# UltronAI/Depth-VO-Feat

Measured on AMD Instinct MI355X. Metric: KITTI 256x832 stereo-seq samples/sec fwd+bwd, higher is better.
Workload: dtype f32

## Files before the change

depth-vo-feat_amd/csrc/conv.hip:

```cpp
#include "dvf_common.h"
#include "conv_op.h"
#include "conv_pipe_host.h"
#include "conv_gather.h"
#include "conv_wgrad.h"
#include "wgrad_pipe.h"

namespace {

__device__ __forceinline__ float act_grad(float g, float yv, int act, float alpha, float beta) {
    if (act == DVF_ACT_RELU) return (yv > 0.f) ? g : 0.f;
    if (act == DVF_ACT_SIGMOID_AFFINE) {
        const float sg = (yv - beta) / alpha;
        return g * alpha * sg * (1.f - sg);
    }
    return g;
}

template <bool VEC>
__global__ __launch_bounds__(256) void act_bwd_kernel(const float *__restrict__ dy, const float *__restrict__ y,
                                                      float *__restrict__ dpre, float *dbias, int C, int HW, int act,
                                                      float alpha, float beta, int chunks, float *part = nullptr, int nper = 0) {
    __shared__ float red[4];
    const int plane = blockIdx.x / chunks, chunk = blockIdx.x - plane * chunks;
    const int c = plane % C;
// ... 224 lines not shown
    else rc = launch_gather_ck<1, 1>(a, pl, st);
    if (rc) return rc;
    dvf_plan_note(DVF_K_GATHER, pl.MT, pl.NT, 1, 2 * pl.CKH, 0, a.KS, 1, 1, 256, (int)pl.lds, a.out_mode | (a.ncls << 4));
    return finish_output(a, pl.reduce_kpar, ws, io.out, st);
}

enum FwdDirect { FWD_NONE, FWD_HEAD, FWD_HEAD_WIDE, FWD_DCONVT };
FwdDirect fwd_direct(const dvf_conv_desc *d, int nseg) {
    if (dvf_head_applicable(d, nseg)) return FWD_HEAD;
    if (dvf_head_wide_applicable(d, nseg)) return FWD_HEAD_WIDE;
    if (dvf_dconvt_applicable(d, nseg)) return FWD_DCONVT;
    return FWD_NONE;
}

int fwd_unpacked(const dvf_conv_desc *d, const ConvOp &op, const ConvIO &io, const int *seg_channels, int nseg, const float *w,
                 float *ws, int64_t ws_floats, hipStream_t st) {
    switch (fwd_direct(d, nseg)) {
        case FWD_HEAD: return dvf_head_fwd(d, io.in[0], w, io.bias, io.out, st);
        case FWD_HEAD_WIDE: return dvf_head_fwd_segs(d, io.in, seg_channels, nseg, w, io.bias, io.out, st);
        case FWD_DCONVT: return dvf_dconvt_fwd(d, io.in[0], w, io.bias, io.out, st);
        case FWD_NONE: break;
    }
    GatherPlan pl;
    const int rc = plan_gather(op, pl);
    return rc ? rc : run_gather(op, pl, io, w, ws, ws_floats, st);
}

int dgrad_unpacked(const dvf_conv_desc *d, const ConvOp &op, const ConvIO &io, const float *w, float *ws, int64_t ws_floats,
                   hipStream_t st) {
    if (dvf_head_seg_dgrad_applicable(d, op.M))
        return dvf_head_seg_dgrad(d, io.in[0], w, io.out, op.m_base, op.M, st, io.mask);
    GatherPlan pl;
    const int rc = plan_gather(op, pl);
    return rc ? rc : run_gather(op, pl, io, w, ws, ws_floats, st);
}

int64_t unpacked_ws_floats(const ConvOp &op, bool direct) {
    if (direct) return 0;
    GatherPlan pl;
    const int rc = plan_gather(op, pl);
    return rc ? rc : pl.ws_floats;
}

struct DgradSeg {
    int s, off;
    ConvOp op;
    bool packed;
    PipePlan plan;
    int64_t packed_off;
};

template <class F>
int for_each_dgrad_seg(const dvf_conv_desc *d, const int *seg_channels, int nseg, bool use_pipe, F visit) {
    DgradSeg v;
    v.off = 0; v.packed_off = 0;
    for (v.s = 0; v.s < nseg; ++v.s) {
        int rc = make_dgrad_op(d, v.off, seg_channels[v.s], v.op);
        v.packed = false;
        if (use_pipe) {
            if (rc) return rc;
            rc = plan_pipe(v.op, v.plan);
            if (rc && rc != DVF_ERR_UNSUPPORTED) return rc;
            v.packed = !rc;
        }
        rc = visit(v);
        if (rc) return rc;
        if (v.packed) v.packed_off += v.plan.packed_floats;
        v.off += seg_channels[v.s];
    }
    return DVF_OK;
}

int64_t conv_sizes(const dvf_conv_desc *d, const int *seg_channels, int nseg, int op_kind, bool want_ws) {
    int rc = check_desc(d);
    if (rc) return rc;
    rc = check_segs(d, seg_channels, nseg);
    if (rc) return rc;
    if (op_kind == 0) {
        if (!want_ws && dvf_dconvt_applicable(d, nseg)) return DVF_ERR_UNSUPPORTED;
        ConvOp op;
        PipePlan pl;
        rc = make_fwd_op(d, seg_channels, nseg, op);
        if (rc) return rc;
        rc = plan_pipe(op, pl);
        if (rc == DVF_ERR_UNSUPPORTED && want_ws) return unpacked_ws_floats(op, fwd_direct(d, nseg) != FWD_NONE);
        return rc ? rc : (want_ws ? pl.ws_floats : pl.packed_floats);
    }
    if (op_kind != 1) return DVF_ERR_INVALID_ARG;
    int64_t total = 0, wmax = 0;
    int nsup = 0;
    rc = for_each_dgrad_seg(d, seg_channels, nseg, true, [&](const DgradSeg &v) -> int {
        int64_t wf = 0;
        if (v.packed) {
            total += v.plan.packed_floats;
            wf = v.plan.ws_floats;
            ++nsup;
        } else if (want_ws) {
            wf = unpacked_ws_floats(v.op, dvf_head_seg_dgrad_applicable(d, v.op.M));
            if (wf < 0) return (int)wf;
        }
        wmax = wf > wmax ? wf : wmax;
        return DVF_OK;
    });
    if (rc) return rc;
    if (!nsup && !want_ws) return DVF_ERR_UNSUPPORTED;
    return want_ws ? wmax : total;
}

WgradArgs wgrad_args(const dvf_conv_desc *d, const float *const *in_segs, const int *seg_channels, int s, const float *dpre,
                     float *dw) {
    int off = 0;
    for (int i = 0; i < s; ++i) off += seg_channels[i];
    const int segc = s < 0 ? d->C_in : seg_channels[s];
    WgradArgs a{};
    a.KK = d->KH * d->KW; a.KH = d->KH; a.KW = d->KW; a.N = d->N; a.S = d->stride; a.pad = d->pad; a.G = dw;
    if (!d->transposed) {
        a.P = dpre; a.PCtot = d->C_out; a.m_base = 0; a.M = d->C_out; a.GH = d->H_out; a.GW = d->W_out;
        a.Q = s < 0 ? nullptr : in_segs[s]; a.QCtot = segc; a.q_base = 0; a.Cq = segc; a.QH = d->H_in; a.QW = d->W_in;
        a.g_mstride = (int64_t)d->C_in * a.KK; a.g_mbase = 0; a.g_cbase = off;
    } else {
        a.P = in_segs[s]; a.PCtot = segc; a.m_base = 0; a.M = segc; a.GH = d->H_in; a.GW = d->W_in;
        a.Q = dpre; a.QCtot = d->C_out; a.q_base = 0; a.Cq = d->C_out; a.QH = d->H_out; a.QW = d->W_out;
        a.g_mstride = (int64_t)d->C_out * a.KK; a.g_mbase = off; a.g_cbase = 0;
    }
    return a;
}

struct WgradPipePlan {
    WgpArgs w;
    int MT, NTW, TILE, nblocks;
    size_t lds;
    int64_t ws_floats;
};

int plan_wgrad_pipe(const WgradArgs &o, const int *qsegc, int nseg, bool aligned16, bool want_bias, WgradPipePlan &pl) {
    static const bool off = dvf_tune("DVF_WG_PIPE") && atoi(dvf_tune("DVF_WG_PIPE")) == 0;
    if (off) return DVF_ERR_UNSUPPORTED;
    const int T = o.KH * o.KW;
    if ((o.S != 1 && o.S != 2) || T > 128 || o.pad < 0 || o.pad > 4) return DVF_ERR_UNSUPPORTED;
    if ((int64_t)o.N * o.PCtot * o.GH * o.GW * 4 >= ((int64_t)1 << 31) - 16 ||
        nseg < 1 || nseg > DVF_MAX_SEGS)
        return DVF_ERR_UNSUPPORTED;
    WgpArgs &w = pl.w;
    w = WgpArgs{};
    for (int s = 0; s < nseg; ++s) {
        if ((int64_t)o.N * qsegc[s] * o.QH * o.QW * 4 >= ((int64_t)1 << 31) - 16) return DVF_ERR_UNSUPPORTED;
        w.segC[s] = qsegc[s];
    }
    w.nseg = nseg;
    w.PCtot = o.PCtot; w.m_base = o.m_base; w.M = o.M; w.Cq = o.Cq;
    w.g_mstride = o.g_mstride; w.g_mbase = o.g_mbase; w.g_cbase = o.g_cbase; w.KK = o.KK; w.KH = o.KH; w.KW = o.KW;
    w.N = o.N; w.GH = o.GH; w.GW = o.GW; w.QH = o.QH; w.QW = o.QW; w.S = o.S; w.pad = o.pad;
    w.XA = (o.pad + 3) & ~3;
    w.RSq = roundup(w.XA + (WGP_BW - 1) * o.S + o.KW - o.pad, 4);
    w.PHq = (WGP_BH - 1) * o.S + o.KH;
    w.x4 = (o.GW % 4 == 0 && o.QW % 4 == 0 && aligned16) ? 1 : 0;
    if (const char *e = dvf_tune("DVF_WG_X4")) w.x4 = w.x4 && atoi(e) != 0;
    const int piece = w.x4 ? 256 : 64;
    w.NPIq = cdiv(w.PHq * w.RSq, piece);
    if (w.NPIq > WGP_MAXQ) return DVF_ERR_UNSUPPORTED;
    w.PSq = w.NPIq * piece + 4;
    static const bool no16 = dvf_tune("DVF_WG_TILE16") && atoi(dvf_tune("DVF_WG_TILE16")) == 0;
    double best_cost = 1e30;
    int TILE = 0, MT = 0, NTW = 0, CK = 0;
    for (int tile = 32; tile >= 16; tile -= 16) {
        if (tile == 16 && no16) break;
        for (int mt = 2; mt >= 1; --mt) {
            if (mt == 2 && o.M <= tile) continue;
            const int pf = (tile * mt / 2) * WGP_PAIR;
            for (int ntw = (tile == 16 ? 4 : 2); ntw >= 1; --ntw) {
                int ckmax = (4 * ntw * tile) / T;
                if (ckmax > o.Cq) ckmax = o.Cq;
                while (ckmax >= 1 && (size_t)2 * (pf + (size_t)(ckmax + 1) * w.PSq) * 4 > WGP_LDS_CAP) --ckmax;
                if (ckmax < 1) continue;
                const int nch = cdiv(o.Cq, ckmax);
                double cost = (double)cdiv(o.M, tile * mt) * nch * mt * ntw * (tile == 32 ? 4 : 1);
                if (tile == 16) cost *= 1.15;
                if (cost < best_cost) { best_cost = cost; TILE = tile; MT = mt; NTW = ntw; CK = cdiv(o.Cq, nch); }
            }
        }
    }
    const int MB = TILE * MT, PF = (MB / 2) * WGP_PAIR;
    if (!NTW) return DVF_ERR_UNSUPPORTED;
    w.CK = CK;
    w.mtiles = cdiv(o.M, MB);
    w.cchunks = cdiv(o.Cq, CK);
    w.tilesX = cdiv(o.GW, WGP_BW);
    w.tilesY = cdiv(o.GH, WGP_BH);
    w.ntiles = o.N * w.tilesX * w.tilesY;
    const int64_t W = (int64_t)w.mtiles * w.cchunks * w.ntiles;
    if (W >= ((int64_t)1 << 30)) return DVF_ERR_UNSUPPORTED;
    w.W = (int)W;
    static const int ncu = [] {
        int dev = 0, n = 0;
        if (hipGetDevice(&dev) != hipSuccess || hipDeviceGetAttribute(&n, hipDeviceAttributeMultiprocessorCount, dev) != hipSuccess || n < 1) n = 256;
        return n;
    }();
    const int nblocks = w.W < ncu ? w.W : ncu;
    w.bias_col = (want_bias && CK * T < 4 * NTW * TILE) ? CK * T : -1;
    w.QSLOTS = CK + (w.bias_col >= 0 ? 1 : 0);
    const size_t lds = (size_t)2 * (PF + (size_t)w.QSLOTS * w.PSq) * 4;
    const int64_t need = wgrad_pipe_slots(w, nblocks) * wgrad_pipe_slot_floats(MT, NTW, TILE);
    pl.MT = MT; pl.NTW = NTW; pl.TILE = TILE; pl.nblocks = nblocks; pl.lds = lds; pl.ws_floats = need;
    return DVF_OK;
}

int run_wgrad_pipe(const WgradPipePlan &pl, const float *P, const float *const *qsegs, float *G, float *dbias, bool *bias_done,
                   float *ws, int64_t ws_floats, hipStream_t st) {
    WgpArgs w = pl.w;
    w.P = P; w.G = G;
    for (int s = 0; s < w.nseg; ++s) w.Q[s] = qsegs[s];
    w.dbias = w.bias_col >= 0 ? dbias : nullptr;
    w.ws = (ws && ws_floats >= pl.ws_floats) ? ws : nullptr;
    if (const char *e = dvf_tune("DVF_WG_DBG")) w.dbg = atoi(e);
    w.stamps = nullptr;
#ifdef DVF_TUNING
    if (dvf_tune("DVF_WG_STAMPS")) {
        if (!g_stamp_buf && hipMalloc(&g_stamp_buf, STAMP_MAX_BLOCKS * 64) != hipSuccess) return DVF_ERR_LAUNCH;
        if ((size_t)pl.nblocks <= STAMP_MAX_BLOCKS) {
            if (hipMemsetAsync(g_stamp_buf, 0, (size_t)pl.nblocks * 64, st) != hipSuccess) return DVF_ERR_LAUNCH;
            w.stamps = g_stamp_buf;
            g_stamp_blocks = pl.nblocks;
        }
    }
#endif
    int rc = dvf_wgrad_pipe_launch(w, pl.MT, pl.NTW, pl.nblocks, pl.lds, st, pl.TILE);
    if (rc == DVF_OK && w.ws) rc = dvf_wgrad_pipe_reduce(w, pl.MT, pl.NTW, pl.nblocks, st, pl.TILE);
    if (rc) return rc;
    dvf_plan_note(DVF_K_WGRAD_PIPE, pl.MT | (pl.TILE << 8), pl.NTW, w.x4 | (w.ws ? 2 : 0), w.CK, w.S, w.NPIq, pl.nblocks, (int)pl.lds,
                  w.KH * w.KW, w.RSq, w.nseg);
    if (bias_done) *bias_done = w.bias_col >= 0;
    return DVF_OK;
}

bool aligned16(const float *p, const float *const *q, int n) {
    uintptr_t v = reinterpret_cast<uintptr_t>(p);
    for (int s = 0; s < n; ++s) v |= reinterpret_cast<uintptr_t>(q[s]);
    return (v & 15) == 0;
}

int wgrad_route(const dvf_conv_desc *d, const float *const *in_segs, const int *seg_channels, int nseg, const float *dpre,
                float *dw, int accumulate, float *dbias, bool *bias_done, float *ws, int64_t ws_floats, hipStream_t st) {
    *bias_done = false;
    if (dvf_head_applicable(d, nseg)) {
        if (!in_segs[0]) return DVF_ERR_INVALID_ARG;
        return dvf_head_wgrad(d, in_segs[0], dpre, dw, accumulate, st, ws, ws_floats);
    }
    if (!accumulate && hipMemsetAsync(dw, 0, sizeof(float) * (size_t)d->C_in * d->C_out * d->KH * d->KW, st) != hipSuccess)
        return DVF_ERR_LAUNCH;
    for (int s = 0; s < nseg; ++s)
        if (!in_segs[s]) return DVF_ERR_INVALID_ARG;
    WgradPipePlan pp;
    if (!d->transposed) {
        const WgradArgs a = wgrad_args(d, in_segs, seg_channels, -1, dpre, dw);
        int rc = plan_wgrad_pipe(a, seg_channels, nseg, aligned16(dpre, in_segs, nseg), dbias != nullptr, pp);
        if (!rc) rc = run_wgrad_pipe(pp, dpre, in_segs, dw, dbias, bias_done, ws, ws_floats, st);
        if (rc != DVF_ERR_UNSUPPORTED) return rc;
    }
    for (int s = 0; s < nseg; ++s) {
        WgradArgs a = wgrad_args(d, in_segs, seg_channels, s, dpre, dw);
        int rc = DVF_ERR_UNSUPPORTED;
        if (d->transposed) {
            rc = plan_wgrad_pipe(a, &d->C_out, 1, aligned16(a.P, &dpre, 1), false, pp);
            if (!rc) rc = run_wgrad_pipe(pp, a.P, &dpre, dw, nullptr, nullptr, ws, ws_floats, st);
        }
        if (rc == DVF_ERR_UNSUPPORTED) {
            WgradRegPlan rp;
            rc = plan_wgrad_reg(a, rp);
            if (!rc) rc = launch_wgrad_reg(a, rp, st);
        }
        if (rc) return rc;
    }
    return DVF_OK;
}

}

extern "C" {

int64_t dvf_conv2d_wgrad_ws_floats(const dvf_conv_desc *d, const int *seg_channels, int nseg) {
    int rc = check_desc(d);
    if (rc) return rc;
    rc = check_segs(d, seg_channels, nseg);
    if (rc) return rc;
    int64_t need = 0;
    if (dvf_head_applicable(d, nseg)) {
        need = dvf_head_wgrad_ws_floats(d);
    } else {
        const float *const none[DVF_MAX_SEGS] = {};
        WgradPipePlan pp;
        auto plan = [&](int s, const int *qsegc, int qnseg) {
            const WgradArgs a = wgrad_args(d, none, seg_channels, s, nullptr, nullptr);
            if (plan_wgrad_pipe(a, qsegc, qnseg, true, false, pp) == DVF_OK && pp.ws_floats > need) need = pp.ws_floats;
        };
        if (!d->transposed) plan(-1, seg_channels, nseg);
        else for (int s = 0; s < nseg; ++s) plan(s, &d->C_out, 1);
    }
    const int64_t nb = dvf_act_bwd_ws_floats(d->N, d->C_out, d->H_out * d->W_out);
    return need > nb ? need : nb;
}

int dvf_conv2d_wgrad(const dvf_conv_desc *d, const float *const *in_segs, const int *seg_channels, int nseg,
                     const float *dpre, float *dw, int accumulate, float *dbias, int accumulate_dbias, float *ws,
                     int64_t ws_floats, void *stream) {
    if (!d) return DVF_ERR_INVALID_ARG;
    hipStream_t st = dvf_stream(stream);
    if (dbias && !accumulate_dbias &&
        hipMemsetAsync(dbias, 0, sizeof(float) * (size_t)(d->C_out > 0 ? d->C_out : 0), st) != hipSuccess)
        return DVF_ERR_LAUNCH;
    dvf_plan_reset();
    int rc = check_desc(d);
    if (rc) return rc;
    rc = check_segs(d, seg_channels, nseg);
    if (rc) return rc;
    if (!in_segs || !dpre || !dw) return DVF_ERR_INVALID_ARG;
    bool done = false;
    rc = wgrad_route(d, in_segs, seg_channels, nseg, dpre, dw, accumulate, dbias, &done, ws, ws_floats, st);
    if (rc || done || !dbias) return rc;
    return dvf_act_bwd(dpre, nullptr, nullptr, dbias, d->N, d->C_out, d->H_out * d->W_out, DVF_ACT_NONE, 1.f, 0.f, 1, ws, ws_floats, stream);
}

static int act_bwd_chunks(int N, int C, int HW, bool has_bias) {
    int chunks = (HW + 8191) / 8192;
    const int64_t planes = (int64_t)N * C;
    while (chunks > 1 && planes * chunks > 16384) chunks >>= 1;
    while (planes * chunks < 1024 && HW / (chunks * 2) >= 1024 && (!has_bias || (int64_t)N * chunks * 2 <= 128)) chunks *= 2;
// ... 179 lines not shown
```

depth-vo-feat_amd/csrc/wgrad_pipe.hip:

```cpp
#include "wgrad_pipe.h"
#include "conv_pipe.h"

namespace {

using dvfp::f32x16;
using dvfp::lds_void_t;
using dvfp::OOB;
using dvfp::tensor_rsrc;

constexpr int WGP_THREADS = 512;

template <int LB>
__device__ __forceinline__ void dma_piece(__amdgpu_buffer_rsrc_t r, float *dst, unsigned voff, unsigned soff) {
    if constexpr (LB == 16) __builtin_amdgcn_raw_ptr_buffer_load_lds(r, (lds_void_t *)dst, 16, voff, soff, 0, 0);
    else __builtin_amdgcn_raw_ptr_buffer_load_lds(r, (lds_void_t *)dst, 4, voff, soff, 0, 0);
}
typedef float f4 __attribute__((ext_vector_type(4)));

template <int MT, int NTW, int S, int TILE>
__global__ __launch_bounds__(WGP_THREADS) void wgrad_pipe_kernel(const WgpArgs a) {
    constexpr int MB = TILE * MT, PF = (MB / 2) * WGP_PAIR;
    constexpr int KQ = 64 / TILE;
    extern __shared__ __attribute__((aligned(16))) float smem[];
    const int tid = threadIdx.x, lane = tid & 63, nl = lane & (TILE - 1), kh = lane / TILE;
    const int wave = __builtin_amdgcn_readfirstlane(tid >> 6);
    const int stage_floats = PF + a.QSLOTS * a.PSq;
    const int nb = gridDim.x, b = blockIdx.x;
    const int w0 = (int)(((int64_t)a.W * b) / nb), w1 = (int)(((int64_t)a.W * (b + 1)) / nb);
    const int nitems = w1 - w0;
    if (nitems <= 0) return;
    if (DVF_DBG(a, 32)) return;
    unsigned long long t_entry = 0, r_entry = 0;
    DVF_STAMP(a, t_entry);
    DVF_STAMP_RT(a, r_entry);
    int mc = w0 / a.ntiles;
    int tile = w0 - mc * a.ntiles;

    if (wave >= 4) {
        __builtin_amdgcn_s_setprio(3);
        const int pidx = wave - 4;
        const int planeP = a.GH * a.GW, planeQ = a.QH * a.QW;
        unsigned p_off[4];
        int p_row[4], p_col[4];
#pragma unroll
        for (int kk = 0; kk < 4; ++kk) {
            int ch, row, col;
            if (a.x4) { ch = lane >> 5; row = (lane >> 3) & 3; col = (lane & 7) << 2; }
            else { ch = kk >> 1; row = ((kk & 1) << 1) + (lane >> 5); col = lane & 31; }
            p_off[kk] = (unsigned)(ch * planeP + row * a.GW + col) << 2;
            p_row[kk] = row;
            p_col[kk] = col;
        }
        int q_row[WGP_MAXQ], q_col[WGP_MAXQ];
        {
            const int per_row = a.x4 ? (a.RSq >> 2) : a.RSq;
#pragma unroll
            for (int kk = 0; kk < WGP_MAXQ; ++kk) {
                q_row[kk] = -(1 << 20);
                q_col[kk] = 0;
                if (kk < a.NPIq) {
                    const int L = (kk << 6) + lane;
                    const int row = L / per_row, col = L - row * per_row;
                    q_row[kk] = row < a.PHq ? row : -(1 << 20);
                    q_col[kk] = a.x4 ? (col << 2) : col;
                }
            }
        }
        const __amdgpu_buffer_rsrc_t rs_zero_dbg = __builtin_amdgcn_make_buffer_rsrc(const_cast<float *>(a.P), 0, 0, 0x00020000);
        const __amdgpu_buffer_rsrc_t rs_p = DVF_DBG(a, 512) ? rs_zero_dbg : tensor_rsrc(a.P);
        const int txy = a.tilesX * a.tilesY;
        int n = tile / txy;
        int tY = (tile - n * txy) / a.tilesX;
        int tX = tile - n * txy - tY * a.tilesX;
        auto U = [](int v) __attribute__((always_inline)) { return __builtin_amdgcn_readfirstlane(v); };
        static_assert(DVF_MAX_SEGS == 5, "segment table below");
        const int sc0 = U(a.segC[0]), sc1 = U(a.nseg > 1 ? a.segC[1] : 0), sc2 = U(a.nseg > 2 ? a.segC[2] : 0),
                  sc3 = U(a.nseg > 3 ? a.segC[3] : 0), sc4 = U(a.nseg > 4 ? a.segC[4] : 0);
        const float *const q0 = a.Q[0], *const q1 = a.Q[a.nseg > 1 ? 1 : 0], *const q2 = a.Q[a.nseg > 2 ? 2 : 0],
                    *const q3 = a.Q[a.nseg > 3 ? 3 : 0], *const q4 = a.Q[a.nseg > 4 ? 4 : 0];
        auto segc_of = [&](int sg) __attribute__((always_inline)) { return sg == 0 ? sc0 : sg == 1 ? sc1 : sg == 2 ? sc2 : sg == 3 ? sc3 : sc4; };
        auto segp_of = [&](int sg) __attribute__((always_inline)) { return sg == 0 ? q0 : sg == 1 ? q1 : sg == 2 ? q2 : sg == 3 ? q3 : q4; };
        const int PSqu = U(a.PSq), NPIu = U(a.NPIq), CKu = U(a.CK), Cqu = U(a.Cq), mtu = U(a.mtiles), sfl = U(stage_floats);
        const unsigned planeQb = (unsigned)U(planeQ << 2), planePb = (unsigned)U(planeP << 2);
        unsigned long long w_p = 0, w_v = 0, w_q = 0;
        auto issue = [&](int st, auto npc, auto exactc) __attribute__((always_inline)) {
            constexpr int NP = decltype(npc)::value;
            constexpr bool EXACT = decltype(exactc)::value;
            float *Pst = smem + st * sfl;
            float *Qst = Pst + PF;
            const int mb = mc % mtu, cb = mc / mtu;
            const int m0 = mb * MB, c0 = cb * CKu;
            const int nch = min(CKu, Cqu - c0);
            const int gy0 = tY * WGP_BH, gx0 = tX * WGP_BW;
            if (DVF_DBG(a, 1)) return;
            unsigned long long s0 = 0, s1 = 0, s2 = 0, s3 = 0;
            DVF_STAMP(a, s0);
            if (!DVF_DBG(a, 2048)) {
                const int mrem = a.M - m0;
                const int npairs = min(MB / 2, (mrem + 1) >> 1);
                unsigned soff = ((unsigned)((n * a.PCtot + a.m_base + m0) * planeP + gy0 * a.GW + gx0) << 2) + (unsigned)(2 * pidx) * planePb;
                unsigned pvo[4];
#pragma unroll
                for (int kk = 0; kk < 4; ++kk)
                    pvo[kk] = ((gy0 + p_row[kk] < a.GH) && (gx0 + p_col[kk] < a.GW)) ? p_off[kk] : OOB;
                float *dst = Pst + pidx * WGP_PAIR;
                for (int pp = pidx; pp < npairs; pp += 4) {
                    const bool odd_tail = (2 * pp + 1 >= mrem);
                    if (a.x4) {
                        const unsigned vo = (odd_tail && lane >= 32) ? OOB : pvo[0];
                        dma_piece<16>(rs_p, dst, vo, soff);
                    } else {
#pragma unroll
                        for (int kk = 0; kk < 4; ++kk) {
                            const unsigned vo = (odd_tail && kk >= 2) ? OOB : pvo[kk];
                            dma_piece<4>(rs_p, dst + (kk << 6), vo, soff);
                        }
                    }
                    soff += 8u * planePb;
                    dst += 4 * WGP_PAIR;
                }
            }
            DVF_STAMP(a, s1);
            if (!DVF_DBG(a, 4096)) {
                const int qy0 = gy0 * S - a.pad, qx0 = gx0 * S - a.XA;
                unsigned qvo[NP];
#pragma unroll
                for (int kk = 0; kk < NP; ++kk) {
                    qvo[kk] = OOB;
                    if (EXACT || kk < NPIu) {
                        const int iy = qy0 + q_row[kk], ix = qx0 + q_col[kk];
                        const bool ok = (iy >= 0) && (iy < a.QH) && (ix >= 0) && (ix < a.QW);
                        qvo[kk] = ok ? ((unsigned)(iy * a.QW + ix) << 2) : OOB;
                    }
                }
                DVF_STAMP(a, s2);
                int ci = pidx, seg = 0, seg_first = 0;
                float *dst = Qst + pidx * PSqu;
                while (ci < nch) {
                    const int vc = c0 + ci;
                    while (vc >= seg_first + segc_of(seg)) { seg_first += segc_of(seg); ++seg; }
                    const int sgc = segc_of(seg);
                    const int ci_end = min(nch, seg_first + sgc - c0);
                    const __amdgpu_buffer_rsrc_t rs_q = DVF_DBG(a, 1024) ? rs_zero_dbg : tensor_rsrc(segp_of(seg));
                    unsigned soff = (unsigned)(n * sgc + (vc - seg_first)) * planeQb;
                    for (; ci < ci_end; ci += 4) {
#pragma unroll
                        for (int kk = 0; kk < NP; ++kk)
                            if (EXACT || kk < NPIu) {
                                if (a.x4) dma_piece<16>(rs_q, dst + (kk << 8), qvo[kk], soff);
                                else dma_piece<4>(rs_q, dst + (kk << 6), qvo[kk], soff);
                            }
                        soff += 4u * planeQb;
                        dst += 4 * PSqu;
                    }
                }
                DVF_STAMP(a, s3);
                w_p += s1 - s0; w_v += s2 - s1; w_q += s3 - s2;
            }
        };
        auto advance = [&]() __attribute__((always_inline)) {
            ++tile;
            if (++tX == a.tilesX) {
                tX = 0;
                if (++tY == a.tilesY) { tY = 0; ++n; }
            }
            if (tile == a.ntiles) { tile = 0; n = 0; ++mc; }
        };
        if (DVF_DBG(a, 64)) return;
        unsigned long long p0 = 0, p1 = 0, p2 = 0, p3 = 0, w_vm = 0, w_bar = 0, w_iss = 0;
        auto item_loop = [&](auto npc, auto exactc) __attribute__((always_inline)) {
            issue(0, npc, exactc);
            advance();
            for (int x = 0; x < nitems; ++x) {
                DVF_STAMP(a, p0);
                asm volatile("s_waitcnt vmcnt(0)" ::: "memory");
                DVF_STAMP(a, p1);
                __builtin_amdgcn_s_barrier();
                DVF_STAMP(a, p2);
                if (x + 1 < nitems) {
                    issue((x + 1) & 1, npc, exactc);
                    advance();
                }
                DVF_STAMP(a, p3);
                w_vm += p1 - p0; w_bar += p2 - p1; w_iss += p3 - p2;
            }
        };
        using std::integral_constant;
        switch (NPIu) {
            case 1: item_loop(integral_constant<int, 1>{}, std::true_type{}); break;
            case 2: item_loop(integral_constant<int, 2>{}, std::true_type{}); break;
            case 3: item_loop(integral_constant<int, 3>{}, std::true_type{}); break;
            case 4: item_loop(integral_constant<int, 4>{}, std::true_type{}); break;
            default:
                if (NPIu <= 8) item_loop(integral_constant<int, 8>{}, std::false_type{});
                else item_loop(integral_constant<int, WGP_MAXQ>{}, std::false_type{});
        }
        if (DVF_STAMPS_ON && a.stamps && pidx == 0 && lane == 0) {
            a.stamps[8 * b + 5] = w_vm; a.stamps[8 * b + 6] = w_bar; a.stamps[8 * b + 7] = w_iss;
            if (DVF_DBG(a, 256)) { a.stamps[8 * b + 5] = w_p; a.stamps[8 * b + 6] = w_v; a.stamps[8 * b + 7] = w_q; }
        }
        return;
    }

    const int T = a.KH * a.KW;
    int loff[NTW], cjv[NTW], tjv[NTW];
#pragma unroll
    for (int u = 0; u < NTW; ++u) {
        const int j = (wave * NTW + u) * TILE + nl;
        const int cj = j / T, tj = j - cj * T, ta = tj / a.KW, tb = tj - ta * a.KW;
        const bool in_chunk = cj < a.CK;
        loff[u] = in_chunk ? cj * a.PSq + ta * a.RSq + tb + (a.XA - a.pad) : 0;
        cjv[u] = in_chunk ? cj : -1;
        tjv[u] = tj;
        if (j == a.bias_col) {
            loff[u] = a.CK * a.PSq;
            cjv[u] = -2;
        }
    }
    if (a.bias_col >= 0) {
        for (int e = tid; e < a.PSq; e += 256) {
            smem[PF + a.CK * a.PSq + e] = 1.f;
            smem[stage_floats + PF + a.CK * a.PSq + e] = 1.f;
        }
    }
    constexpr int NACC = TILE == 32 ? 16 : 4;
    typedef float accv __attribute__((ext_vector_type(NACC)));
    accv acc[MT][NTW];
#pragma unroll
    for (int m = 0; m < MT; ++m)
#pragma unroll
        for (int u = 0; u < NTW; ++u)
#pragma unroll
            for (int r = 0; r < NACC; ++r) acc[m][u][r] = 0.f;

    auto consume = [&](int st, int vy, int vg) {
        const float *Pst = smem + st * stage_floats;
        const float *Qst = Pst + PF;
        const float *ap = Pst + ((nl >> 1) * WGP_PAIR + (nl & 1) * 128 + 4 * kh);
        const float *bp[NTW];
#pragma unroll
        for (int u = 0; u < NTW; ++u) bp[u] = Qst + loff[u] + 4 * kh * S;
        f4 A[2][MT];
        float B[2][NTW][4];
        constexpr int GP = 4 * KQ, GPR = WGP_BW / GP;
        int ly = 0, ltq = 0;
        auto load = [&](auto bufc) {
            constexpr int buf = decltype(bufc)::value;
            const int y = ly, tq = ltq;
            if (++ltq == vg) { ltq = 0; ++ly; }
            const float *ay = ap + y * 32 + GP * tq;
#pragma unroll
            for (int m = 0; m < MT; ++m) A[buf][m] = *reinterpret_cast<const f4 *>(ay + m * (TILE / 2) * WGP_PAIR);
            const int qo = (y * S) * a.RSq + GP * tq * S;
#pragma unroll
            for (int u = 0; u < NTW; ++u) {
                const float *bg = bp[u] + qo;
#pragma unroll
                for (int i = 0; i < 4; ++i) B[buf][u][i] = bg[i * S];
            }
        };
        auto mma = [&](auto bufc) {
            constexpr int buf = decltype(bufc)::value;
#pragma unroll
            for (int i = 0; i < 4; ++i)
#pragma unroll
                for (int m = 0; m < MT; ++m)
#pragma unroll
                    for (int u = 0; u < NTW; ++u) {
                        if constexpr (TILE == 32)
                            acc[m][u] = __builtin_amdgcn_mfma_f32_32x32x2f32(A[buf][m][i], B[buf][u][i], acc[m][u], 0, 0, 0);
                        else
                            acc[m][u] = __builtin_amdgcn_mfma_f32_16x16x4f32(A[buf][m][i], B[buf][u][i], acc[m][u], 0, 0, 0);
                    }
        };
        using B0 = std::integral_constant<int, 0>;
        using B1 = std::integral_constant<int, 1>;
        static_assert(GPR * GP == WGP_BW, "groups tile a row");
        const int NGv = vy * vg;
        load(B0{});
        for (int it = 0; it < NGv; it += 2) {
            load(B1{});
            mma(B0{});
            if (it + 2 < NGv) load(B0{});
            mma(B1{});
        }
    };
    auto flush = [&](int mcv) {
        if (a.ws) {
            float *slab = a.ws + (int64_t)(b + mcv) * (MB * 4 * NTW * TILE) + wave * 64 + lane;
#pragma unroll
            for (int m = 0; m < MT; ++m)
#pragma unroll
                for (int u = 0; u < NTW; ++u)
#pragma unroll
                    for (int r = 0; r < NACC; ++r) {
                        slab[((m * NTW + u) * NACC + r) * 256] = DVF_DBG(a, 8) ? 0.f : acc[m][u][r];
                        acc[m][u][r] = 0.f;
                    }
            return;
        }
        const int mb = mcv % a.mtiles, cb = mcv / a.mtiles;
        const int m0 = mb * MB, c0 = cb * a.CK;
        const int nch = min(a.CK, a.Cq - c0);
        const bool full_m = m0 + MB <= a.M;
        auto row_of = [](int m, int r) { return TILE == 32 ? m * 32 + (r & 3) + 8 * (r >> 2) : m * 16 + r; };
#pragma unroll
        for (int u = 0; u < NTW; ++u) {
            const bool colok = cjv[u] >= 0 && cjv[u] < nch && !DVF_DBG(a, 8);
            float *gl = a.G + (int64_t)(a.g_mbase + m0 + 4 * kh) * a.g_mstride + (int64_t)(a.g_cbase + c0 + cjv[u]) * a.KK + tjv[u];
            if (colok) {
#pragma unroll
                for (int m = 0; m < MT; ++m)
#pragma unroll
                    for (int r = 0; r < NACC; ++r) {
                        const int ml = row_of(m, r);
                        if (full_m || m0 + 4 * kh + ml < a.M) atomicAdd(gl + (int64_t)ml * a.g_mstride, acc[m][u][r]);
                    }
            }
            if (cjv[u] == -2 && cb == 0) {
                float *bl = a.dbias + m0 + 4 * kh;
#pragma unroll
                for (int m = 0; m < MT; ++m)
#pragma unroll
                    for (int r = 0; r < NACC; ++r) {
                        const int ml = row_of(m, r);
                        if (full_m || m0 + 4 * kh + ml < a.M) atomicAdd(bl + ml, acc[m][u][r]);
                    }
            }
#pragma unroll
            for (int m = 0; m < MT; ++m)
#pragma unroll
                for (int r = 0; r < NACC; ++r) acc[m][u][r] = 0.f;
        }
    };
    if (DVF_DBG(a, 64)) return;
    unsigned long long t_loop0 = 0, t_loop1 = 0, tb0 = 0, tb1 = 0, tf0 = 0, tf1 = 0, w_bar = 0, w_flush = 0;
    DVF_STAMP(a, t_loop0);
    int ctY, ctX;
    {
        const int txy = a.tilesX * a.tilesY, r = tile % txy;
        ctY = r / a.tilesX;
        ctX = r - ctY * a.tilesX;
    }
    constexpr int GPX = 4 * (64 / TILE);
    for (int x = 0; x < nitems; ++x) {
        const int vy = min(WGP_BH, a.GH - ctY * WGP_BH);
        const int vg = (min(WGP_BW, a.GW - ctX * WGP_BW) + GPX - 1) / GPX;
        if (++ctX == a.tilesX) { ctX = 0; if (++ctY == a.tilesY) ctY = 0; }
        DVF_STAMP(a, tb0);
        asm volatile("s_waitcnt lgkmcnt(0)\n\ts_barrier" ::: "memory");
        DVF_STAMP(a, tb1);
        w_bar += tb1 - tb0;
        if (!DVF_DBG(a, 4)) consume(x & 1, vy, vg);
        int mc_next = mc;
        if (++tile == a.ntiles) { tile = 0; ++mc_next; }
        if ((x == nitems - 1 || mc_next != mc) && !DVF_DBG(a, 128)) {
            DVF_STAMP(a, tf0);
            flush(mc);
            DVF_STAMP(a, tf1);
            w_flush += tf1 - tf0;
        }
        mc = mc_next;
    }
    DVF_STAMP(a, t_loop1);
    if (DVF_STAMPS_ON && a.stamps && wave == 0) {
        unsigned long long r_end = 0;
        asm volatile("s_waitcnt vmcnt(0)" ::: "memory");
        DVF_STAMP_RT(a, r_end);
        if (lane == 0) {
            unsigned long long *o = a.stamps + 8 * b;
            o[0] = t_loop0 - t_entry; o[1] = t_loop1 - t_loop0; o[2] = w_bar; o[3] = w_flush; o[4] = r_end - r_entry;
        }
    }
}

template <int MT, int NTW, int S, int TILE>
// ... 87 lines not shown
```

Before: 647.3.

## Shrink wgrad LDS tiles for small planes and precompute DMA offsets per loop

When the gradient plane is smaller than the fixed block tile, the weight-gradient pipe kernel now sizes its LDS patch (RSq, PHq, NPIq) from the effective width and height. For small deep layers this cuts the number of DMA pieces issued per channel. Per-lane buffer offsets for P and Q are computed once per item loop instead of on every issue. Interior tiles and single-tile layers reuse them through a shifted base pointer, and only edge tiles redo the bounds masks. The change adds zero-fill of the skew padding, a separate tail-pair path for P, and specialised loops for the x4 and non-x4 cases. This makes the addressing more complex and carries a correctness risk where reads reach past the DMA region.

```diff
diff --git a/depth-vo-feat_amd/csrc/conv.hip b/depth-vo-feat_amd/csrc/conv.hip
--- a/depth-vo-feat_amd/csrc/conv.hip
+++ b/depth-vo-feat_amd/csrc/conv.hip
@@ -400,14 +400,29 @@
     w.g_mstride = o.g_mstride; w.g_mbase = o.g_mbase; w.g_cbase = o.g_cbase; w.KK = o.KK; w.KH = o.KH; w.KW = o.KW;
     w.N = o.N; w.GH = o.GH; w.GW = o.GW; w.QH = o.QH; w.QW = o.QW; w.S = o.S; w.pad = o.pad;
     w.XA = (o.pad + 3) & ~3;
-    w.RSq = roundup(w.XA + (WGP_BW - 1) * o.S + o.KW - o.pad, 4);
-    w.PHq = (WGP_BH - 1) * o.S + o.KH;
+    const int BWe = o.GW < WGP_BW ? o.GW : WGP_BW;
+    int BHe = o.GH < WGP_BH ? o.GH : WGP_BH;
+    if (BHe < WGP_BH && (BHe & 1)) ++BHe;
+    w.RSq = roundup(w.XA + (BWe - 1) * o.S + o.KW - o.pad, 4);
+    w.PHq = (BHe - 1) * o.S + o.KH;
     w.x4 = (o.GW % 4 == 0 && o.QW % 4 == 0 && aligned16) ? 1 : 0;
     if (const char *e = dvf_tune("DVF_WG_X4")) w.x4 = w.x4 && atoi(e) != 0;
     const int piece = w.x4 ? 256 : 64;
     w.NPIq = cdiv(w.PHq * w.RSq, piece);
     if (w.NPIq > WGP_MAXQ) return DVF_ERR_UNSUPPORTED;
-    w.PSq = w.NPIq * piece + 4;
+    const int reach = (w.PHq - 1) * w.RSq + (w.XA - o.pad) + o.KW - 1 + (roundup(BWe, 16) - 1) * o.S;
+    const int over = reach + 1 - w.NPIq * piece;
+    if (over > 32) return DVF_ERR_UNSUPPORTED;
+    w.PSq = w.NPIq * piece + (over > 0 ? 36 : 4);
+    const int NPI_full = cdiv(((WGP_BH - 1) * o.S + o.KH) * roundup(w.XA + (WGP_BW - 1) * o.S + o.KW - o.pad, 4), piece);
+    if (NPI_full > WGP_MAXQ) return DVF_ERR_UNSUPPORTED;
+    const int PSq_full = NPI_full * piece + 4;
+    if (w.PSq > PSq_full) {
+        w.RSq = roundup(w.XA + (WGP_BW - 1) * o.S + o.KW - o.pad, 4);
+        w.PHq = (WGP_BH - 1) * o.S + o.KH;
+        w.NPIq = NPI_full;
+        w.PSq = PSq_full;
+    }
     static const bool no16 = dvf_tune("DVF_WG_TILE16") && atoi(dvf_tune("DVF_WG_TILE16")) == 0;
     double best_cost = 1e30;
     int TILE = 0, MT = 0, NTW = 0, CK = 0;
@@ -419,7 +434,7 @@
             for (int ntw = (tile == 16 ? 4 : 2); ntw >= 1; --ntw) {
                 int ckmax = (4 * ntw * tile) / T;
                 if (ckmax > o.Cq) ckmax = o.Cq;
-                while (ckmax >= 1 && (size_t)2 * (pf + (size_t)(ckmax + 1) * w.PSq) * 4 > WGP_LDS_CAP) --ckmax;
+                while (ckmax >= 1 && (size_t)2 * (pf + (size_t)(ckmax + 1) * PSq_full) * 4 > WGP_LDS_CAP) --ckmax;
                 if (ckmax < 1) continue;
                 const int nch = cdiv(o.Cq, ckmax);
                 double cost = (double)cdiv(o.M, tile * mt) * nch * mt * ntw * (tile == 32 ? 4 : 1);
diff --git a/depth-vo-feat_amd/csrc/wgrad_pipe.hip b/depth-vo-feat_amd/csrc/wgrad_pipe.hip
--- a/depth-vo-feat_amd/csrc/wgrad_pipe.hip
+++ b/depth-vo-feat_amd/csrc/wgrad_pipe.hip
@@ -82,58 +82,59 @@
         auto segp_of = [&](int sg) __attribute__((always_inline)) { return sg == 0 ? q0 : sg == 1 ? q1 : sg == 2 ? q2 : sg == 3 ? q3 : q4; };
         const int PSqu = U(a.PSq), NPIu = U(a.NPIq), CKu = U(a.CK), Cqu = U(a.Cq), mtu = U(a.mtiles), sfl = U(stage_floats);
         const unsigned planeQb = (unsigned)U(planeQ << 2), planePb = (unsigned)U(planeP << 2);
+        const int x4u = U(a.x4), GHu = U(a.GH), GWu = U(a.GW), QHu = U(a.QH), QWu = U(a.QW), PHu = U(a.PHq), RSu = U(a.RSq);
+        const bool one_tile = U(a.tilesX == 1 && a.tilesY == 1);
+        int mb = U(mc % a.mtiles), cb = U(mc / a.mtiles);
         unsigned long long w_p = 0, w_v = 0, w_q = 0;
-        auto issue = [&](int st, auto npc, auto exactc) __attribute__((always_inline)) {
+        auto emit = [&](int st, auto npc, auto exactc, const unsigned (&pv)[4], unsigned pvt, const auto &qv, int q_org,
+                        unsigned long long s1) __attribute__((always_inline)) {
             constexpr int NP = decltype(npc)::value;
             constexpr bool EXACT = decltype(exactc)::value;
             float *Pst = smem + st * sfl;
             float *Qst = Pst + PF;
-            const int mb = mc % mtu, cb = mc / mtu;
             const int m0 = mb * MB, c0 = cb * CKu;
             const int nch = min(CKu, Cqu - c0);
             const int gy0 = tY * WGP_BH, gx0 = tX * WGP_BW;
-            if (DVF_DBG(a, 1)) return;
-            unsigned long long s0 = 0, s1 = 0, s2 = 0, s3 = 0;
-            DVF_STAMP(a, s0);
+            unsigned long long s2 = 0, s3 = 0, s4 = 0;
+            DVF_STAMP(a, s2);
             if (!DVF_DBG(a, 2048)) {
                 const int mrem = a.M - m0;
-                const int npairs = min(MB / 2, (mrem + 1) >> 1);
-                unsigned soff = ((unsigned)((n * a.PCtot + a.m_base + m0) * planeP + gy0 * a.GW + gx0) << 2) + (unsigned)(2 * pidx) * planePb;
-                unsigned pvo[4];
-#pragma unroll
-                for (int kk = 0; kk < 4; ++kk)
-                    pvo[kk] = ((gy0 + p_row[kk] < a.GH) && (gx0 + p_col[kk] < a.GW)) ? p_off[kk] : OOB;
+                const int nfull = min(MB / 2, mrem >> 1);
+                const bool tail = (mrem & 1) && (mrem >> 1) < MB / 2 && ((mrem >> 1) & 3) == pidx;
+                const unsigned base = (unsigned)((n * a.PCtot + a.m_base + m0) * planeP + gy0 * GWu + gx0) << 2;
+                const bool upper = GHu - gy0 > 2;
+                unsigned soff = base + (unsigned)(2 * pidx) * planePb;
                 float *dst = Pst + pidx * WGP_PAIR;
-                for (int pp = pidx; pp < npairs; pp += 4) {
-                    const bool odd_tail = (2 * pp + 1 >= mrem);
-                    if (a.x4) {
-                        const unsigned vo = (odd_tail && lane >= 32) ? OOB : pvo[0];
-                        dma_piece<16>(rs_p, dst, vo, soff);
-                    } else {
-#pragma unroll
-                        for (int kk = 0; kk < 4; ++kk) {
-                            const unsigned vo = (odd_tail && kk >= 2) ? OOB : pvo[kk];
-                            dma_piece<4>(rs_p, dst + (kk << 6), vo, soff);
-                        }
-                    }
-                    soff += 8u * planePb;
-                    dst += 4 * WGP_PAIR;
+                if (x4u) {
+                    for (int pp = pidx; pp < nfull; pp += 4) {
+                        dma_piece<16>(rs_p, dst, pv[0], soff);
+                        soff += 8u * planePb;
+                        dst += 4 * WGP_PAIR;
+                    }
+                    if (tail) dma_piece<16>(rs_p, Pst + (mrem >> 1) * WGP_PAIR, pvt, base + (unsigned)(mrem - 1) * planePb);
+                } else if (upper) {
+                    for (int pp = pidx; pp < nfull; pp += 4) {
+#pragma unroll
+                        for (int kk = 0; kk < 4; ++kk) dma_piece<4>(rs_p, dst + (kk << 6), pv[kk], soff);
+                        soff += 8u * planePb;
+                        dst += 4 * WGP_PAIR;
+                    }
+                    if (tail) {
+                        dma_piece<4>(rs_p, Pst + (mrem >> 1) * WGP_PAIR, pv[0], base + (unsigned)(mrem - 1) * planePb);
+                        dma_piece<4>(rs_p, Pst + (mrem >> 1) * WGP_PAIR + 64, pv[1], base + (unsigned)(mrem - 1) * planePb);
+                    }
+                } else {
+                    for (int pp = pidx; pp < nfull; pp += 4) {
+                        dma_piece<4>(rs_p, dst, pv[0], soff);
+                        dma_piece<4>(rs_p, dst + 128, pv[2], soff);
+                        soff += 8u * planePb;
+                        dst += 4 * WGP_PAIR;
+                    }
+                    if (tail) dma_piece<4>(rs_p, Pst + (mrem >> 1) * WGP_PAIR, pv[0], base + (unsigned)(mrem - 1) * planePb);
                 }
             }
-            DVF_STAMP(a, s1);
+            DVF_STAMP(a, s3);
             if (!DVF_DBG(a, 4096)) {
-                const int qy0 = gy0 * S - a.pad, qx0 = gx0 * S - a.XA;
-                unsigned qvo[NP];
-#pragma unroll
-                for (int kk = 0; kk < NP; ++kk) {
-                    qvo[kk] = OOB;
-                    if (EXACT || kk < NPIu) {
-                        const int iy = qy0 + q_row[kk], ix = qx0 + q_col[kk];
-                        const bool ok = (iy >= 0) && (iy < a.QH) && (ix >= 0) && (ix < a.QW);
-                        qvo[kk] = ok ? ((unsigned)(iy * a.QW + ix) << 2) : OOB;
-                    }
-                }
-                DVF_STAMP(a, s2);
                 int ci = pidx, seg = 0, seg_first = 0;
                 float *dst = Qst + pidx * PSqu;
                 while (ci < nch) {
@@ -141,22 +142,57 @@
                     while (vc >= seg_first + segc_of(seg)) { seg_first += segc_of(seg); ++seg; }
                     const int sgc = segc_of(seg);
                     const int ci_end = min(nch, seg_first + sgc - c0);
-                    const __amdgpu_buffer_rsrc_t rs_q = DVF_DBG(a, 1024) ? rs_zero_dbg : tensor_rsrc(segp_of(seg));
+                    const __amdgpu_buffer_rsrc_t rs_q = DVF_DBG(a, 1024) ? rs_zero_dbg : tensor_rsrc(segp_of(seg) + q_org);
                     unsigned soff = (unsigned)(n * sgc + (vc - seg_first)) * planeQb;
-                    for (; ci < ci_end; ci += 4) {
-#pragma unroll
-                        for (int kk = 0; kk < NP; ++kk)
-                            if (EXACT || kk < NPIu) {
-                                if (a.x4) dma_piece<16>(rs_q, dst + (kk << 8), qvo[kk], soff);
-                                else dma_piece<4>(rs_q, dst + (kk << 6), qvo[kk], soff);
-                            }
-                        soff += 4u * planeQb;
-                        dst += 4 * PSqu;
+                    if (x4u) {
+                        for (; ci < ci_end; ci += 4) {
+#pragma unroll
+                            for (int kk = 0; kk < NP; ++kk)
+                                if (EXACT || kk < NPIu) dma_piece<16>(rs_q, dst + (kk << 8), qv[kk], soff);
+                            soff += 4u * planeQb;
+                            dst += 4 * PSqu;
+                        }
+                    } else {
+                        for (; ci < ci_end; ci += 4) {
+#pragma unroll
+                            for (int kk = 0; kk < NP; ++kk)
+                                if (EXACT || kk < NPIu) dma_piece<4>(rs_q, dst + (kk << 6), qv[kk], soff);
+                            soff += 4u * planeQb;
+                            dst += 4 * PSqu;
+                        }
                     }
                 }
-                DVF_STAMP(a, s3);
-                w_p += s1 - s0; w_v += s2 - s1; w_q += s3 - s2;
-            }
+            }
+            DVF_STAMP(a, s4);
+            w_p += s3 - s2; w_v += s2 - s1; w_q += s4 - s3;
+        };
+        auto issue = [&](int st, auto npc, auto exactc, const unsigned (&psx)[4], unsigned ptx, const auto &qsx) __attribute__((always_inline)) {
+            constexpr int NP = decltype(npc)::value;
+            constexpr bool EXACT = decltype(exactc)::value;
+            if (DVF_DBG(a, 1)) return;
+            unsigned long long s1 = 0;
+            DVF_STAMP(a, s1);
+            const int gy0 = tY * WGP_BH, gx0 = tX * WGP_BW;
+            const int qy0 = gy0 * S - a.pad, qx0 = gx0 * S - a.XA;
+            const bool inside = gy0 + WGP_BH <= GHu && gx0 + WGP_BW <= GWu && qy0 >= 0 && qy0 + PHu <= QHu && qx0 >= 0 &&
+                                qx0 + RSu <= QWu;
+            if (one_tile || inside) {
+                emit(st, npc, exactc, psx, ptx, qsx, one_tile ? 0 : qy0 * QWu + qx0, s1);
+                return;
+            }
+            const int vyP = GHu - gy0, vxP = GWu - gx0;
+            const int ylo = max(0, -qy0), ny = max(0, min(PHu, QHu - qy0) - ylo);
+            const int xlo = max(0, -qx0), nx = max(0, min(RSu, QWu - qx0) - xlo);
+            unsigned pvo[4], qvo[NP];
+#pragma unroll
+            for (int kk = 0; kk < 4; ++kk) pvo[kk] = (p_row[kk] < vyP && p_col[kk] < vxP) ? psx[kk] : OOB;
+#pragma unroll
+            for (int kk = 0; kk < NP; ++kk) {
+                qvo[kk] = OOB;
+                if (EXACT || kk < NPIu)
+                    qvo[kk] = ((unsigned)(q_row[kk] - ylo) < (unsigned)ny && (unsigned)(q_col[kk] - xlo) < (unsigned)nx) ? qsx[kk] : OOB;
+            }
+            emit(st, npc, exactc, pvo, lane >= 32 ? OOB : pvo[0], qvo, qy0 * QWu + qx0, s1);
         };
         auto advance = [&]() __attribute__((always_inline)) {
             ++tile;
@@ -164,12 +200,32 @@
                 tX = 0;
                 if (++tY == a.tilesY) { tY = 0; ++n; }
             }
-            if (tile == a.ntiles) { tile = 0; n = 0; ++mc; }
+            if (tile == a.ntiles) {
+                tile = 0; n = 0; ++mc;
+                if (++mb == mtu) { mb = 0; ++cb; }
+            }
         };
         if (DVF_DBG(a, 64)) return;
         unsigned long long p0 = 0, p1 = 0, p2 = 0, p3 = 0, w_vm = 0, w_bar = 0, w_iss = 0;
         auto item_loop = [&](auto npc, auto exactc) __attribute__((always_inline)) {
-            issue(0, npc, exactc);
+            constexpr int NP = decltype(npc)::value;
+            constexpr bool EXACT = decltype(exactc)::value;
+            unsigned psx[4], qsx[NP];
+#pragma unroll
+            for (int kk = 0; kk < 4; ++kk)
+                psx[kk] = (!one_tile || (p_row[kk] < GHu && p_col[kk] < GWu)) ? p_off[kk] : OOB;
+            const unsigned ptx = lane >= 32 ? OOB : psx[0];
+#pragma unroll
+            for (int kk = 0; kk < NP; ++kk) {
+                qsx[kk] = OOB;
+                if (EXACT || kk < NPIu) {
+                    const int iy = q_row[kk] - (one_tile ? a.pad : 0), ix = q_col[kk] - (one_tile ? a.XA : 0);
+                    const bool ok = one_tile ? (iy >= 0) && (iy < QHu) && (ix >= 0) && (ix < QWu) : q_row[kk] >= 0;
+                    qsx[kk] = ok ? ((unsigned)(iy * QWu + ix) << 2) : OOB;
+                }
+            }
+            auto issue_st = [&](int st) __attribute__((always_inline)) { issue(st, npc, exactc, psx, ptx, qsx); };
+            issue_st(0);
             advance();
             for (int x = 0; x < nitems; ++x) {
                 DVF_STAMP(a, p0);
@@ -178,7 +234,7 @@
                 __builtin_amdgcn_s_barrier();
                 DVF_STAMP(a, p2);
                 if (x + 1 < nitems) {
-                    issue((x + 1) & 1, npc, exactc);
+                    issue_st((x + 1) & 1);
                     advance();
                 }
                 DVF_STAMP(a, p3);
@@ -222,6 +278,15 @@
             smem[PF + a.CK * a.PSq + e] = 1.f;
             smem[stage_floats + PF + a.CK * a.PSq + e] = 1.f;
         }
+    }
+    {
+        const int dma_floats = a.NPIq * (a.x4 ? 256 : 64), skew = a.PSq - dma_floats;
+        if (skew > 4)
+            for (int e = tid; e < a.CK * skew; e += 256) {
+                const int ci = e / skew, o = dma_floats + (e - ci * skew);
+                smem[PF + ci * a.PSq + o] = 0.f;
+                smem[stage_floats + PF + ci * a.PSq + o] = 0.f;
+            }
     }
     constexpr int NACC = TILE == 32 ? 16 : 4;
     typedef float accv __attribute__((ext_vector_type(NACC)));
```

Result: no change. 653.1, median of 6 (+0.9%).
